# GregDMeyer/dynamite

Measured on AMD Instinct MI355X. Metric: matrix-free H|psi> Gamplitudes/s, random-field Heisenberg, higher is better.
Workload: dtype f64 (complex128)

## Files before the change

dynamite_amd/_lib.py:

```python
import ctypes as C
import os

import numpy as np

from . import build as _build

_HERE = os.path.dirname(os.path.abspath(__file__))

i64p = C.POINTER(C.c_int64)
f64p = C.POINTER(C.c_double)
vp = C.c_void_p


class Subspace(C.Structure):
    _fields_ = [("type", C.c_int32), ("L", C.c_int64), ("space", C.c_int64), ("k", C.c_int64),
                ("ld_nchoosek", C.c_int64), ("nchoosek", i64p), ("dim", C.c_int64),
                ("state_map", i64p), ("rmap_indices", i64p), ("rmap_states", i64p), ("vec_swizzle", C.c_int32),
                ("site_perm", C.POINTER(C.c_int8))]


class Partition(C.Structure):
    _fields_ = [("rank", C.c_int32), ("nranks", C.c_int32)]


# ... 17 lines not shown
LP_COUNT = 9
LP_NAMES = ["tile_real_k0", "tile_real", "tile_cplx", "tile_kvar_real", "tile_kvar_cplx", "gather_real",
            "gather_kvar_real", "gather_cplx", "gather_kvar_cplx"]
LP_KVAR, LP_CPLX, LP_GATHER = (3, 4, 6, 8), (2, 4, 7, 8), (5, 6, 7, 8)


class DevQuad(C.Structure):
    _fields_ = [("mask_tile", C.c_uint32), ("mask_loc", C.c_uint32), ("src", C.c_uint32),
                ("nslots", C.c_uint32), ("sign_tile", C.c_uint32 * 4), ("sign_ext", C.c_uint64 * 4),
                ("coeff", C.c_double * 4)]


class DevPass(C.Structure):
    _fields_ = [("nseg", C.c_int32), ("seg_off", C.c_int32 * MAXSEG), ("seg_len", C.c_int32 * MAXSEG),
                ("seg_pos", C.c_int32 * MAXSEG), ("nbseg", C.c_int32), ("bseg_off", C.c_int32 * MAXBSEG),
                ("bseg_len", C.c_int32 * MAXBSEG), ("bseg_pos", C.c_int32 * MAXBSEG),
                ("sign_base", C.c_uint64), ("accumulate", C.c_int32), ("need_tile", C.c_int32),
                ("has_diag", C.c_int32), ("cache_policy", C.c_int32), ("dext_begin", C.c_uint32), ("dext_end", C.c_uint32),
                ("dbucket", C.c_uint32 * (MAXR + 1)), ("loop", C.c_uint32 * (LP_COUNT + 1)),
                ("nquads", C.c_int32), ("n_eff", C.c_int32), ("quads", vp), ("dot_out", vp), ("zinit", vp), ("zscale", C.c_double), ("zinit2", vp), ("z2re", C.c_double), ("z2im", C.c_double),
                ("tile_bits", C.c_int32), ("log_rows", C.c_int32),
                ("swz_shift", C.c_int32), ("swz_xor_y", C.c_uint32), ("swz_xor_src", C.c_uint32), ("block_offset", C.c_uint32),
                ("pos_tmask", C.c_uint32), ("dtile", vp), ("tabs", vp), ("tabvals", vp), ("tab_loop", C.c_uint32 * 3),
                ("pad_tab", C.c_uint32), ("gbucket", C.c_uint32 * (MAXR + 1)), ("pad_g", C.c_uint32)]


class DevTab(C.Structure):
    _fields_ = [("mask_tile", C.c_uint32), ("mask_loc", C.c_uint32), ("src", C.c_uint32), ("first", C.c_uint32),
                ("z_tile", C.c_uint32), ("flags", C.c_uint32), ("tpos", C.c_uint32), ("twid", C.c_uint32),
                ("epos", C.c_uint32), ("ewid", C.c_uint32), ("z_ext", C.c_uint64), ("ik", C.c_uint64),
                ("ksign", C.c_uint32), ("nbits", C.c_uint32)]


class DevFlip(C.Structure):
    _fields_ = [("mask_tile", C.c_uint32), ("mask_pos", C.c_uint32), ("p0", C.c_uint32), ("p1", C.c_uint32),
                ("pad", C.c_uint32 * 2), ("c", C.c_double)]


FL_COUNT = 4
FL_NAMES = ["tile_thread", "tile_k", "gather_uniform", "gather_boundary"]


class Xfer(C.Structure):
    _fields_ = [("partner", C.c_int32), ("pass_id", C.c_int32), ("offset", C.c_int64), ("count", C.c_int64)]


MAT_DEFAULT, MAT_FORCE_GATHER, MAT_USE_GLDS, MAT_HOST_ONLY = 0, 1, 2, 4
# ... 46 lines not shown
    "dnm_mat_local_part_bits": (C.c_int, [vp, C.POINTER(C.c_int), C.POINTER(C.c_int)]),
    "dnm_mat_mult_window_local": (C.c_int, [vp, vp, vp, vp]),
    "dnm_mat_mult_window_remote": (C.c_int, [vp, vp, C.c_int64, C.c_int64, vp, vp]),
    "dnm_mat_window_local_rows": (C.c_int, [vp, C.c_int64, C.c_int64, C.c_int, C.c_int, C.POINTER(C.c_int64), C.POINTER(C.c_int), vp]),
    "dnm_mat_mult_window_rows": (C.c_int, [vp, vp, C.c_int64, C.c_int64, vp, C.c_int64, C.c_int64, vp]),
    "dnm_mat_destroy": (C.c_int, [vp]),
    "dnm_mat_sizes": (C.c_int, [vp, i64p, i64p, i64p, i64p]),
    "dnm_mat_precompute_diagonal": (C.c_int, [vp, vp]),
    "dnm_mat_get_diagonal": (C.c_int, [vp, f64p, vp]),
    "dnm_mat_mult": (C.c_int, [vp, vp, vp, vp]),
    "dnm_mat_norm_inf": (C.c_int, [vp, f64p, vp]),
    "dnm_mat_set_norm": (C.c_int, [vp, C.c_double]),
    "dnm_mat_plan_describe": (C.c_int, [vp, C.c_char_p, C.c_size_t]),
    "dnm_mat_plan_launches": (C.c_int, [vp, C.POINTER(C.c_int)]),
    "dnm_mat_plan_counts": (C.c_int, [vp] + [C.POINTER(C.c_int)] * 6),
    "dnm_mat_export_dtile": (C.c_int, [vp, C.c_int, C.c_int, f64p, C.c_int64]),
    "dnm_mat_export_tabs": (C.c_int, [vp, C.c_int, C.c_int, vp, C.c_size_t, C.c_int, C.POINTER(C.c_int), f64p, C.c_int64, i64p]),
    "dnm_mat_export_pass": (C.c_int, [vp, C.c_int, C.c_int, vp, C.c_size_t, vp, C.c_size_t, C.c_int,
                                      C.POINTER(C.c_int)]),
    "dnm_mat_export_flip": (C.c_int, [vp, C.c_int, C.c_int, vp, C.c_size_t, C.c_int, C.POINTER(C.c_int),
                                      C.POINTER(C.c_uint32), f64p]),
    "dnm_mat_export_flip_pass": (C.c_int, [vp, C.c_int, C.c_int, vp, C.c_size_t, vp, C.c_size_t, C.c_int,
                                           C.POINTER(C.c_int), f64p, C.c_int64, i64p]),
    "dnm_mat_ownership": (C.c_int, [vp, i64p, i64p]),
    "dnm_mat_column_window": (C.c_int, [vp, i64p, i64p, vp]),
    "dnm_mat_column_chunks": (C.c_int, [vp, C.c_int, C.POINTER(C.c_uint8), C.c_int64, vp]),
    "dnm_mat_mult_window": (C.c_int, [vp, vp, C.c_int64, C.c_int64, vp, vp]),
    "dnm_mat_exchange_plan": (C.c_int, [vp, C.POINTER(C.c_int), C.POINTER(Xfer), C.POINTER(C.c_int),
                                        C.POINTER(Xfer)]),
    "dnm_mat_mult_dot": (C.c_int, [vp, vp, vp, f64p, vp]),
    "dnm_mat_mult_lanczos": (C.c_int, [vp, vp, vp, vp, C.c_double, f64p, vp]),
    "dnm_mat_mult_local": (C.c_int, [vp, vp, vp, vp]),
    "dnm_mat_mult_remote": (C.c_int, [vp, C.c_int32, vp, vp, vp]),
    "dnm_vec_set": (C.c_int, [vp, C.c_int64, C.c_double, C.c_double, vp]),
    "dnm_vec_copy": (C.c_int, [vp, vp, C.c_int64, vp]),
    "dnm_vec_scale": (C.c_int, [vp, C.c_int64, C.c_double, C.c_double, vp]),
    "dnm_vec_axpby": (C.c_int, [vp, vp, C.c_int64, C.c_double, C.c_double, C.c_double, C.c_double, vp]),
    "dnm_vec_dot": (C.c_int, [vp, vp, C.c_int64, f64p, vp]),
    "dnm_vec_norm2": (C.c_int, [vp, C.c_int64, f64p, vp]),
    "dnm_vec_set_random": (C.c_int, [vp, C.c_int64, C.c_uint64, C.c_int64, vp]),
    "dnm_vec_mdot": (C.c_int, [vp, C.c_int64, C.c_int, vp, C.c_int64, f64p, vp]),
    "dnm_vec_maxpy": (C.c_int, [vp, vp, C.c_int64, C.c_int, C.c_int64, f64p, vp]),
    "dnm_vec_basis_update": (C.c_int, [vp, C.c_int64, C.c_int, C.c_int, C.c_int64, f64p, vp]),
    "dnm_workspace_bytes": (C.c_int, [C.POINTER(C.c_size_t)]),
    "dnm_release_workspace": (C.c_int, []),
    "dnm_mat_is_real_packed": (C.c_int, [C.c_void_p, C.POINTER(C.c_int)]),
# ... 77 lines not shown
```

dynamite_amd/csrc/mat.cpp:

```cpp
#include "passes.h"
#include "vec_api.h"
#include "row_fused.h"

#include <algorithm>
#include <cstring>

namespace dnm {

static thread_local std::string g_err;

void set_error(const char *fmt, ...) {
  char buf[1024];
  va_list ap;
  va_start(ap, fmt);
  vsnprintf(buf, sizeof(buf), fmt, ap);
  va_end(ap);
  g_err = buf;
}

int DevBuf::alloc(size_t nbytes) {
  release();
  if (nbytes == 0) nbytes = 16;
  DNM_HIP(hipMalloc(&p, nbytes));
  bytes = nbytes;
// ... 98 lines not shown
      dev.state_map = (const int64_t *)d_smap.p;
      dev.rmap_states = (const int64_t *)d_rstates.p;
      if (!rind.empty()) {
        DNM_TRY(d_rind.upload(rind.data(), rind.size() * 8));
        dev.rmap_indices = (const int64_t *)d_rind.p;
      }
      if (!bucket.empty()) {
        DNM_TRY(d_bucket.upload(bucket.data(), bucket.size() * 8));
        dev.bucket = (const int64_t *)d_bucket.p;
      }
    }
  }
  return 0;
}

template <class T>
static int upload_to(DevBuf &buf, const std::vector<T> &v, const T **dev) {
  DNM_TRY(buf.upload(v.data(), v.size() * sizeof(T)));
  *dev = (const T *)buf.p;
  return 0;
}
int PassRecords::upload() {
  DNM_TRY(upload_to(d_quads, quads, &desc.quads));
  if (!dtile.empty()) DNM_TRY(upload_to(d_dtile, dtile, &desc.dtile));
  if (!tabs.empty()) DNM_TRY(upload_to(d_tabs, tabs, &desc.tabs));
  if (!tabs.empty()) DNM_TRY(upload_to(d_tabvals, tabvals, &desc.tabvals));
  if (is_reduced) DNM_TRY(upload_to(d_flips, flips.empty() ? std::vector<DevFlip>(1) : flips, &flip.recs));
  return 0;
}

static hipStream_t S(void *stream) { return (hipStream_t)stream; }

struct PassCall {
  const void *zinit = nullptr, *zinit2 = nullptr;
  double zscale = 0.0, z2re = 0.0, z2im = 0.0;
  double *dot_out = nullptr;
  uint32_t block_offset = 0;
  unsigned nparts = 1;
};

static int launch_pass(const dnm_mat *A, const PassOnDevice &p, const PassCall &c, const void *x, void *y,
                       const void *xr, hipStream_t st) {
  DevPass d = p.runs().desc;
  d.zinit = c.zinit; d.zscale = c.zscale;
  d.zinit2 = c.zinit2; d.z2re = c.z2re; d.z2im = c.z2im;
  d.dot_out = c.dot_out;
  d.block_offset = c.block_offset;
// ... 6 lines not shown
}

static int export_lookup(const dnm_mat *A, int remote, int idx, const PassOnDevice **p) {
  DNM_CHECK(A, "null argument");
  const auto &v = remote ? A->remote_passes : A->local_passes;
  DNM_CHECK(idx >= 0 && idx < (int)v.size(), "pass index out of range");
  *p = v[idx].get();
  return 0;
}
template <class T>
static int export_copy(const std::vector<T> &v, void *out, size_t item, int64_t room, const char *type, const char *full,
                       bool strict = false) {
  if (!out || (v.empty() && !strict)) return 0;
  DNM_CHECK(item == sizeof(T), "%s size mismatch (%zu vs %zu)", type, item, sizeof(T));
  DNM_CHECK(room >= (int64_t)v.size(), "%s buffer too small", full);
  if (!v.empty()) memcpy(out, v.data(), v.size() * sizeof(T));
  return 0;
}
static int export_records(const PassRecords &r, void *desc_out, size_t desc_bytes, void *quads_out, size_t quad_bytes,
                          int max_quads, int *nquads, bool strict) {
  *nquads = (int)r.quads.size();
  if (desc_out) {
    DNM_CHECK(desc_bytes == sizeof(DevPass), "DevPass size mismatch (%zu vs %zu)", desc_bytes, sizeof(DevPass));
    memcpy(desc_out, &r.desc, sizeof(DevPass));
  }
  return export_copy(r.quads, quads_out, quad_bytes, max_quads, "DevQuad", "record", strict);
}

}

using namespace dnm;

namespace dnm {
std::vector<ScMask> sc_masks(const std::vector<int64_t> &masks, const std::vector<int64_t> &mask_offsets,
                             const std::vector<int64_t> &signs, const std::vector<double> &rcoef, int L, bool xparity) {
  std::vector<ScMask> scm(masks.size());
  for (size_t mi = 0; mi < masks.size(); ++mi) {
    ScMask &e = scm[mi];
    memset(&e, 0, sizeof(e));
    const uint64_t mask = (uint64_t)masks[mi];
    e.dead = __builtin_popcountll(mask) & 1;
    if (xparity && L >= 3 && __builtin_popcountll(mask) == L - 2 && !((mask >> (L - 1)) & 1ull)) {
      const uint64_t miss = ~mask & ((((uint64_t)1 << (L - 1)) - 1));
      const int i = __builtin_ctzll(miss);
      const uint64_t pairbits = ((uint64_t)1 << i) | ((uint64_t)1 << (L - 1));
      bool local = true;
      for (int64_t t = mask_offsets[mi]; t < mask_offsets[mi + 1]; ++t)
// ... 565 lines not shown
    if (cfg.diag_last < 0) cfg.diag_last = cfg.swz ? 1 : 0;
    if (cfg.window_first < 0) {
      int nl = A->op.n;
      for (int r = A->nranks; r > 1; r >>= 1) --nl;
      cfg.window_first = (cfg.swz && nl >= 25) ? 1 : 0;
    }
    if (!tile_config_supported(cfg.B, cfg.logR)) {
      set_error("unsupported tile configuration B=%d logR=%d", cfg.B, cfg.logR);
      return 1;
    }
    DNM_TRY(make_plan(A->op, A->rank, A->nranks, cfg, &A->plan));
    if (flags & DNM_MAT_FORCE_GATHER) A->plan.use_tiled = false;
    DNM_CHECK(!A->real_packed || A->plan.use_tiled, "real-packed operators run on the tiled kernel only (vector too small)");
    if (A->nranks > 1 && !A->plan.use_tiled) {
      A->plan.remote.clear();
      A->plan.sends.clear();
    }
    if (A->plan.use_tiled) {
      DNM_TRY(build_passes(*A, A->plan.local, &A->local_passes));
      DNM_TRY(build_passes(*A, A->plan.remote, &A->remote_passes));
      decide_flip_bonds(A.get());
      for (size_t i = 0; i < A->plan.local.size(); ++i)
        DNM_TRY(build_flip_pass(*A, A->plan.local[i], A->local_passes[i].get()));
      if (!A->host_only)
        for (auto *v : {&A->local_passes, &A->remote_passes})
          for (auto &p : *v) DNM_TRY(p->runs().upload());
    }
  }
  *out = A.release();
  return 0;
}

int dnm_mat_destroy(dnm_mat *A) {
  delete A;
  return 0;
}

int dnm_mat_set_exchange(dnm_mat *A, int scheme, int *chosen) {
  DNM_CHECK(A && chosen, "null argument");
  DNM_CHECK(scheme == DNM_EXCHANGE_AUTO || scheme == DNM_EXCHANGE_PARTNER || scheme == DNM_EXCHANGE_TRANSPOSE,
            "unknown exchange scheme %d", scheme);
  delete A->tr_lo; delete A->tr_hi;
  A->tr_lo = A->tr_hi = nullptr;
  A->tr_f = -1;
  *chosen = DNM_EXCHANGE_PARTNER;
  const int P = A->nranks;
// ... 603 lines not shown
  }
  const int nb = norm_num_blocks(A->rows_local);
  DNM_TRY(A->scratch.alloc((size_t)nb * sizeof(double)));
  DNM_TRY(launch_norm(A->dmsc, A->left.dev, A->right.dev, A->rows_local, A->row0,
                      (double *)A->scratch.p, S(stream)));
  std::vector<double> h(nb);
  DNM_TRY(dnm_memcpy_d2h(h.data(), A->scratch.p, (size_t)nb * sizeof(double), stream));
  double best = 0.0;
  for (double v : h) best = std::max(best, v);
  if (A->nranks == 1) A->nrm = best;
  *nrm = best;
  return 0;
}

int dnm_mat_set_norm(dnm_mat *A, double nrm) {
  DNM_CHECK(A, "null matrix");
  A->nrm = nrm;
  return 0;
}

int dnm_mat_plan_describe(const dnm_mat *A, char *buf, size_t buflen) {
  DNM_CHECK(A && buf && buflen, "null argument");
  std::string s;
  if (A->hypercube) s = A->plan.describe(A->op);
  else if (A->use_sc3) {
    const Sc3Tab &T = A->sc3->ly->host;
    char tmp[512];
    if (A->sc3->tiled && A->sc3->graph)
      snprintf(tmp, sizeof tmp, "SpinConserve two-pass kernels on a bond graph, internal layout [T %d | W %d | Lo %d]: "
               "window pass (%zu workgroups, %d hops in LDS, %d gathered) then lo pass (%zu workgroups, %d hops in LDS, "
               "%d gathered), diagonal %s, coefficients %s\n", T.t, T.w, T.a, A->sc3->permB.size(), A->sc3->op.nldsB,
               A->sc3->op.ngatB, A->sc3->permA.size() / 8, A->sc3->op.nldsA, A->sc3->op.ngatA,
               A->sc3->diag_mode == 2 ? "on the fly" : (A->sc3->diag_mode == 1 ? "cached" : "none"),
               A->sc3->sym ? "real symmetric" : "complex");
    else if (A->sc3->tiled)
      snprintf(tmp, sizeof tmp, "SpinConserve two-pass kernels, internal layout [T %d | W %d | Lo %d]: window pass (%zu "
               "workgroups, %d bonds in LDS, %d gathered) then lo pass (%zu workgroups, %d bonds in LDS, %d gathered), "
               "diagonal %s, coefficients %s\n", T.t, T.w, T.a, A->sc3->permB.size(), T.w - 1,
               __builtin_popcountll(A->sc3->op.bondsB), A->sc3->permA.size() / 8, T.a - 1,
               __builtin_popcountll(A->sc3->op.bondsA),
               A->sc3->diag_mode == 2 ? "on the fly" : (A->sc3->diag_mode == 1 ? "cached" : "none"),
               A->sc3->sym ? "real symmetric" : "complex");
    else
      snprintf(tmp, sizeof tmp, "SpinConserve row kernel, internal layout [T %d | W %d | Lo %d] (positions by table)\n",
               T.t, T.w, T.a);
    s = tmp;
  } else if (A->sc_pair)
// ... 45 lines not shown
                        int *nflips, uint32_t *loops_out, double *dconst) {
  const PassOnDevice *p;
  DNM_CHECK(nflips, "null argument");
  DNM_TRY(export_lookup(A, remote, idx, &p));
  *nflips = p->reduced ? (int)p->reduced->flips.size() : -1;
  if (!p->reduced) return 0;
  if (loops_out) memcpy(loops_out, p->reduced->flip.loop, sizeof(p->reduced->flip.loop));
  if (dconst) *dconst = p->reduced->flip.dconst;
  return export_copy(p->reduced->flips, flips_out, flip_bytes, max_flips, "DevFlip", "record");
}

int dnm_mat_export_flip_pass(const dnm_mat *A, int remote, int idx, void *desc_out, size_t desc_bytes, void *quads_out,
                             size_t quad_bytes, int max_quads, int *nquads, double *dtile_out, int64_t max_dtile,
                             int64_t *ndtile) {
  const PassOnDevice *p;
  DNM_CHECK(nquads && ndtile, "null argument");
  DNM_TRY(export_lookup(A, remote, idx, &p));
  DNM_CHECK(p->reduced, "the pass has no flip-flop form");
  *ndtile = (int64_t)p->reduced->dtile.size();
  DNM_TRY(export_records(*p->reduced, desc_out, desc_bytes, quads_out, quad_bytes, max_quads, nquads, false));
  return export_copy(p->reduced->dtile, dtile_out, sizeof(double), max_dtile, "double", "table");
}

int dnm_mat_plan_counts(const dnm_mat *A, int *n_local_passes, int *n_remote_passes, int *tiled,
                        int *B, int *logR, int *n_loc) {
  DNM_CHECK(A, "null matrix");
  if (n_local_passes) *n_local_passes = (int)A->local_passes.size();
  if (n_remote_passes) *n_remote_passes = (int)A->remote_passes.size();
  if (tiled) *tiled = (A->hypercube && A->plan.use_tiled) ? 1 : 0;
  if (B) *B = A->plan.cfg.B;
  if (logR) *logR = A->plan.cfg.logR;
  if (n_loc) *n_loc = A->plan.n_loc;
  return 0;
}

int dnm_mat_plan_launches(const dnm_mat *A, int *n) {
  DNM_CHECK(A && n, "null argument");
  *n = (A->hypercube && A->plan.use_tiled) ? (int)A->local_passes.size() : 1;
  return 0;
}

}

dnm_mat::~dnm_mat() {
  delete tr_lo;
  delete tr_hi;
// ... 2 lines not shown
```

dynamite_amd/csrc/mat.h:

```cpp
#pragma once

#include <memory>
#include <vector>

#include "kernels.h"
#include "plan.h"
#include "sc3.h"
#include "subspace.h"

namespace dnm {

struct DevBuf {
  void *p = nullptr;
  size_t bytes = 0;
  DevBuf() = default;
  DevBuf(const DevBuf &) = delete;
  DevBuf &operator=(const DevBuf &) = delete;
  ~DevBuf() { release(); }
  int alloc(size_t nbytes);
  int upload(const void *host, size_t nbytes);
  void release();
};

struct SubOwned {
  SubView host{};
  SubView dev{};
  std::vector<int64_t> nck, smap, rind, rstates, bucket;
  DevBuf d_nck, d_smap, d_rind, d_rstates, d_bucket;
  int init(const dnm_subspace *s, bool want_device);
};

struct PassRecords {
  DevPass desc{};
  std::vector<DevQuad> quads;
  std::vector<double> dtile;
  std::vector<DevTab> tabs;
  std::vector<double> tabvals;
  bool is_reduced = false;
  std::vector<DevFlip> flips;
  DevFlipPass flip{};
  DevBuf d_quads, d_dtile, d_tabs, d_tabvals, d_flips;
  int upload();
};

struct PassOnDevice {
  PassRecords whole;
  std::unique_ptr<PassRecords> reduced;
  PassRecords &runs() { return reduced ? *reduced : whole; }
  const PassRecords &runs() const { return reduced ? *reduced : whole; }
  int partner = -1;
  int n_eff = 0;
  int64_t y_off = 0, src_off = 0;
};

struct FlipBond {
  bool ok = false;
  bool exch = false;
  int b0 = 0, b1 = 0;
  double c = 0.0;
};

int rdm_release_scratch();

}
// ... 50 lines not shown
```

dynamite_amd/csrc/matvec_kernels.hip:

```cpp
#include <algorithm>
#include <cstdint>
#include <cstdlib>

#include "kernels.h"

namespace dnm {

typedef double2 c128;

#define GLOBAL_AS __attribute__((address_space(1)))
#define LDS_AS __attribute__((address_space(3)))

typedef double d2v __attribute__((ext_vector_type(2)));

typedef const __attribute__((address_space(4))) DevQuad CQuad;

__device__ __forceinline__ void store_through(c128 *p, double re, double im) {
  d2v v = {re, im};
  asm volatile("global_store_dwordx4 %0, %1, off sc1\n\ts_nop 1" ::"v"(p), "v"(v) : "memory");
}
__device__ __forceinline__ void store_streaming(c128 *p, double re, double im) {
  d2v v = {re, im};
  __builtin_nontemporal_store(v, reinterpret_cast<d2v *>(p));
}
// ... 336 lines not shown
  }
}

#ifndef DNM_WAVES_4ROWS
#define DNM_WAVES_4ROWS 8
#endif
constexpr int tile_waves_per_simd(int B, int LOGR, bool TAB = false) {
  if (TAB) {
    int nt = 1 << (B - LOGR);
    int blocks = (160 * 1024) / (16 << B);
    if (blocks < 1) blocks = 1;
    int w = blocks * nt / 256;
    const int cap = LOGR <= 2 ? 8 : 4;
    return w < 1 ? 1 : (w > cap ? cap : w);
  }
  int nt = 1 << (B - LOGR);
  int blocks = (160 * 1024) / (16 << B);
  if (blocks < 1) blocks = 1;
  int w = blocks * nt / 256;
  const int cap = LOGR <= 2 ? DNM_WAVES_4ROWS : 4;
  return w < 1 ? 1 : (w > cap ? cap : w);
}

template <int B, int LOGR, bool GLDS, int GV, bool PACK, bool TAB, bool FLIP>
__device__ __forceinline__ void tile_pass_body(const DevPass &P, const c128 *__restrict__ x, c128 *__restrict__ y,
                                               const c128 *__restrict__ xr, const DevFlipPass &FP) {
  constexpr int R = 1 << LOGR;
  constexpr int LOGNT = B - LOGR;
  constexpr uint32_t NT = 1u << LOGNT;
  extern __shared__ __attribute__((aligned(16))) unsigned char smem[];
  c128 *tile = reinterpret_cast<c128 *>(smem);

  const uint32_t tid = threadIdx.x;
  DNM_PH(0, 0);
  const uint32_t base = deposit<MAXBSEG>(blockIdx.x + P.block_offset, P.nbseg, P.bseg_off, P.bseg_len, P.bseg_pos);
  const uint32_t dep_t = deposit<MAXSEG>(tid, P.nseg, P.seg_off, P.seg_len, P.seg_pos);
  const uint64_t sbase = P.sign_base | (uint64_t)base;

  const uint32_t skw = (uint32_t)P.swz_shift;
  auto lay = [skw](uint32_t v) -> uint32_t { return skw ? (v ^ (((v >> skw) & ((1u << (skw - 4)) - 1u)) << 4)) : v; };
  RowAddr<R> RA;
  RA.t4 = lay(dep_t) << 4;
  RA.upos = lay(base);
  RA.tmask = P.pos_tmask;
#pragma unroll
  for (int k = 0; k < R; ++k) RA.kpos[k] = lay(deposit<MAXSEG>((uint32_t)k << LOGNT, P.nseg, P.seg_off, P.seg_len, P.seg_pos));
  const uint32_t yx = P.swz_xor_y;
// ... 67 lines not shown

#define DNM_LOOP(LP, KV, CX, GA, KZ) \
  apply_records<R, LOGNT, KV, CX, GA, KZ, PACK>(quads, P.loop[LP], P.loop[LP + 1], ar, ai, tile, RA, x, xr, tid, sbase, skw, P.swz_xor_src)
  if constexpr (GV >= 1) {
    DNM_LOOP(LP_GATHER_REAL, false, false, true, false);
    DNM_LOOP(LP_GATHER_KVAR_REAL, true, false, true, false);
    DNM_LOOP(LP_GATHER_CPLX, false, true, true, false);
    DNM_LOOP(LP_GATHER_KVAR_CPLX, true, true, true, false);
  }
#undef DNM_LOOP
  if constexpr (FLIP)
    flip_gathers<R, LOGNT>((CFlip *)FP.recs, FP.loop[FL_GATHER_U], FP.loop[FL_GATHER_B], FP.loop[FL_GATHER_B + 1], ar, ai, RA,
                           x, tid, sbase);
  c128 *tabl = nullptr;
  if constexpr (TAB) {
    __shared__ __attribute__((aligned(16))) unsigned char tabl_mem[TABL_ENTRIES * 16];
    tabl = reinterpret_cast<c128 *>(tabl_mem);
  }
  if constexpr (TAB)
    apply_tabs<R, LOGNT, true>((CTab *)P.tabs, (const c128 *)P.tabvals, P.tab_loop[1], P.tab_loop[2], ar, ai, tile, RA, x, xr,
                               tid, sbase, skw, P.swz_xor_src, tabl);
  DNM_PH(2, 1);

  double dext = 0.0;
  if (P.has_diag) {
    const uint32_t lane = tid & 63u;
    const uint32_t nterm = (P.dext_end - P.dext_begin) * 4u;
    for (uint32_t t0 = 0; t0 < nterm; t0 += 64u) {
      const uint32_t t = t0 + lane;
      double v = 0.0;
      if (t < nterm) {
        CQuad &Q = quads[P.dext_begin + (t >> 2)];
        const uint32_t j = t & 3u;
        const uint32_t p = (uint32_t)__popcll(sbase & Q.sign_ext[j]) & 1u;
        v = flip_sign(Q.coeff[j], p);
      }
      dext += v;
    }
#pragma unroll
    for (int off = 32; off > 0; off >>= 1) dext += __shfl_xor(dext, off, 64);
  }
  double *cg = nullptr;
  if constexpr (TAB) {
    __shared__ double cg_mem[MAXDGROUPS];
    cg = cg_mem;
    if (P.has_diag) {
      const uint32_t lane = tid & 63u, g0 = P.gbucket[0], g1 = P.gbucket[R];
      for (uint32_t g = g0 + (tid >> 6); g < g1; g += (NT >> 6)) {
        const uint32_t q0 = quads[g].mask_loc, nterm = quads[g].src * 4u;
        double v = 0.0;
        for (uint32_t t0 = 0; t0 < nterm; t0 += 64u) {
          const uint32_t t = t0 + lane;
          if (t < nterm) {
            CQuad &Q = quads[q0 + (t >> 2)];
            const uint32_t j = t & 3u;
            v += flip_sign(Q.coeff[j], (uint32_t)__popcll(sbase & Q.sign_ext[j]) & 1u);
          }
        }
#pragma unroll
        for (int off = 32; off > 0; off >>= 1) v += __shfl_xor(v, off, 64);
        if (lane == 0) cg[g - g0] = v;
      }
    }
  }
  auto diag_part2 = [&]() {
  if (P.has_diag) {
    double D[R];
#pragma unroll
    for (int j = 0; j < R; ++j) D[j] = 0.0;
    D[0] = dext;
    if constexpr (FLIP) D[0] += FP.dconst;
    double dtab[R];
    if (P.dtile) {
#pragma unroll
      for (int k = 0; k < R; ++k) dtab[k] = P.dtile[tid + k * NT];
    }
#pragma unroll
    for (int j = 0; j < R; ++j)
      for (uint32_t q = P.dbucket[j]; q < P.dbucket[j + 1]; ++q) {
        const uint32_t ns = quads[q].nslots;
        double v = slot_amp(quads[q], 0, tid, sbase);
        if (ns > 1) v += slot_amp(quads[q], 1, tid, sbase);
        if (ns > 2) v += slot_amp(quads[q], 2, tid, sbase);
        if (ns > 3) v += slot_amp(quads[q], 3, tid, sbase);
        D[j] += v;
      }
    if constexpr (TAB) {
      const uint32_t g0 = P.gbucket[0];
#pragma unroll
// ... 96 lines not shown
      dn += __shfl_xor(dn, off, 64);
    }
    __shared__ double dred[3 * (NT / 64 > 0 ? NT / 64 : 1)];
    if ((tid & 63u) == 0) {
      dred[3 * (tid >> 6)] = dr;
      dred[3 * (tid >> 6) + 1] = di;
      dred[3 * (tid >> 6) + 2] = dn;
    }
    __syncthreads();
    if (tid == 0) {
      double sr = 0.0, si = 0.0, sn = 0.0;
      for (uint32_t w = 0; w < NT / 64; ++w) {
        sr += dred[3 * w];
        si += dred[3 * w + 1];
        sn += dred[3 * w + 2];
      }
      P.dot_out[3 * (size_t)blockIdx.x] = sr;
      P.dot_out[3 * (size_t)blockIdx.x + 1] = si;
      P.dot_out[3 * (size_t)blockIdx.x + 2] = sn;
    }
  }
}

template <int B, int LOGR, bool GLDS, int GV, bool PACK = false, bool TAB = false>
__global__ void __launch_bounds__(1 << (B - LOGR), tile_waves_per_simd(B, LOGR, TAB))
tile_pass_kernel(const DevPass P, const c128 *__restrict__ x, c128 *__restrict__ y,
                 const c128 *__restrict__ xr) {
  tile_pass_body<B, LOGR, GLDS, GV, PACK, TAB, false>(P, x, y, xr, DevFlipPass{});
}

template <int B, int LOGR, bool GLDS>
__global__ void __launch_bounds__(1 << (B - LOGR), tile_waves_per_simd(B, LOGR, false))
tile_pass_flip_kernel(const DevPass P, const DevFlipPass FP, const c128 *__restrict__ x, c128 *__restrict__ y,
                      const c128 *__restrict__ xr) {
  tile_pass_body<B, LOGR, GLDS, 1, false, false, true>(P, x, y, xr, FP);
}

#ifdef DNM_PHASE_TIMING
}
extern "C" int dnm_debug_phase_buffer(void *buf) {
  unsigned long long *p = (unsigned long long *)buf;
  return hipMemcpyToSymbol(HIP_SYMBOL(dnm::g_phase_buf), &p, sizeof(p)) == hipSuccess ? 0 : 1;
}
namespace dnm {
#endif

template <int B, int LOGR>
static int launch_cfg(const DevPass &P, bool glds, int n_loc, const void *x, void *y,
                      const void *xr, hipStream_t st, unsigned nparts, const DevFlipPass *F) {
  constexpr int NT = 1 << (B - LOGR);
  static const size_t lds_req = []() {
    const char *e = knob("DNM_LDS_KB");
    return e ? (size_t)atoi(e) * 1024 : (size_t)0;
  }();
  const size_t lds = std::max(((size_t)16 << B), lds_req);
  const unsigned grid = (1u << (n_loc - B)) / nparts;
  const int gv = (P.cache_policy & 32) ? 1 : 0;
  using kern_t = void (*)(const DevPass, const c128 *, c128 *, const c128 *);
  kern_t k = nullptr;
  const bool pack = (P.cache_policy & 256) != 0;
  const bool tab = P.tab_loop[2] > 0 || P.gbucket[MAXR] > P.gbucket[0];
  if (F) {
    DNM_CHECK(!pack && !tab && gv == 1, "internal: flip-flop records in a pass that cannot run them");
    using fkern_t = void (*)(const DevPass, const DevFlipPass, const c128 *, c128 *, const c128 *);
    fkern_t fk = glds ? tile_pass_flip_kernel<B, LOGR, true> : tile_pass_flip_kernel<B, LOGR, false>;
    static size_t fattr_done[2] = {0, 0};
    if (fattr_done[glds ? 1 : 0] < lds) {
      DNM_HIP(hipFuncSetAttribute((const void *)fk, hipFuncAttributeMaxDynamicSharedMemorySize, (int)lds));
      fattr_done[glds ? 1 : 0] = lds;
    }
    hipLaunchKernelGGL(fk, dim3(grid), dim3(NT), lds, st, P, *F, (const c128 *)x, (c128 *)y, (const c128 *)xr);
    DNM_HIP(hipGetLastError());
    return 0;
  }
  if (pack) k = tile_pass_kernel<B, LOGR, false, 1, true>;
  else if (tab) k = tile_pass_kernel<B, LOGR, false, 1, false, true>;
  else if (glds) k = tile_pass_kernel<B, LOGR, true, 1>;
  else if (gv == 0) k = tile_pass_kernel<B, LOGR, false, 0>;
  else k = tile_pass_kernel<B, LOGR, false, 1>;
  static size_t attr_done[6] = {0, 0, 0, 0, 0, 0};
  const int slot = pack ? 4 : (tab ? 5 : (glds ? 3 : gv));
  if (attr_done[slot] < lds) {
    DNM_HIP(hipFuncSetAttribute((const void *)k, hipFuncAttributeMaxDynamicSharedMemorySize, (int)lds));
    attr_done[slot] = lds;
  }
  hipLaunchKernelGGL(k, dim3(grid), dim3(NT), lds, st, P, (const c128 *)x, (c128 *)y, (const c128 *)xr);
  DNM_HIP(hipGetLastError());
  return 0;
}

bool tile_config_supported(int B, int logR) {
  switch (B * 16 + logR) {
    case 10 * 16 + 2: case 11 * 16 + 2: case 12 * 16 + 2:
    case 8 * 16 + 2: case 10 * 16 + 3: case 10 * 16 + 4: case 11 * 16 + 3: case 11 * 16 + 4:
    case 12 * 16 + 3: case 12 * 16 + 4: case 13 * 16 + 3: case 13 * 16 + 4:
      return true;
  }
  return false;
}

int launch_tile_pass(const DevPass &P, int B, int logR, bool glds, int n_loc, const void *x,
                     void *y, const void *xr, hipStream_t st, unsigned nparts, const DevFlipPass *F) {
  DNM_CHECK(n_loc >= B, "tile larger than the local vector");
  switch (B * 16 + logR) {
// ... 857 lines not shown
```

dynamite_amd/csrc/passes.cpp:

```cpp
#include "passes.h"

#include <algorithm>
#include <cstring>

namespace dnm {

int build_opform(const dnm_mat &A, OpForm *op) {
  const SubView &l = A.left.host, &r = A.right.host;
  const bool par = l.type == DNM_PARITY;
  const int n = par ? l.L - 1 : l.L;
  op->n = n;
  op->masks.clear();
  const uint64_t ones = n >= 64 ? ~0ull : (((uint64_t)1 << n) - 1);
  for (size_t mi = 0; mi < A.masks.size(); ++mi) {
    const uint64_t mask = (uint64_t)A.masks[mi];
    if (par && (parity64(mask) != (l.space ^ r.space))) continue;
    RowMask rm;
    rm.mask = par ? (mask >> 1) : mask;
    for (int64_t t = A.mask_offsets[mi]; t < A.mask_offsets[mi + 1]; ++t) {
      const uint64_t sg = (uint64_t)A.signs[t];
      RowTerm rt;
      rt.is_imag = parity64(mask & sg);
      double c = A.real_coeffs[t];
      uint64_t s2 = sg;
// ... 537 lines not shown
      DNM_CHECK(it != dterms.end(), "internal: an exchange without a ZZ term on its pair");
      if (it->coeff == a) dterms.erase(it);
      else it->coeff -= a;
      dconst -= a;
      diag_changed = true;
    }
  if (!diag_changed && std::find(skip.begin(), skip.end(), 1) == skip.end()) return 0;
  std::unique_ptr<PassRecords> r(new PassRecords());
  r->is_reduced = true;
  r->desc = d;
  DNM_TRY(emit_records(A, ps, *r, dm ? &dterms : nullptr, skip));
  DNM_CHECK(r->tabs.empty() && r->desc.gbucket[MAXR] == r->desc.gbucket[0],
            "internal: the flip-flop form of a pass has table records or grouped diagonal terms");
  for (int c = 0; c < FL_COUNT; ++c) {
    r->flip.loop[c] = (uint32_t)r->flips.size();
    r->flips.insert(r->flips.end(), fl[c].begin(), fl[c].end());
  }
  r->flip.loop[FL_COUNT] = (uint32_t)r->flips.size();
  r->flip.dconst = dconst;
  out->reduced = std::move(r);
  return 0;
}

}
```

dynamite_amd/csrc/passes.h:

```cpp
#pragma once

#include "mat.h"

namespace dnm {

int build_opform(const dnm_mat &A, OpForm *op);
int pack_opform(OpForm *op);
int build_pass(const dnm_mat &A, const PassSpec &ps, PassOnDevice *out);
void decide_flip_bonds(dnm_mat *A);
int build_flip_pass(const dnm_mat &A, const PassSpec &ps, PassOnDevice *out);

}
```

dynamite_amd/csrc/plan.cpp:

```cpp
#include "plan.h"

#include <algorithm>
#include <cstdlib>
#include <sstream>

namespace dnm {

static int env_int(const char *name, int dflt) {
  const char *v = knob(name);
  if (!v) return dflt;
  return atoi(v);
}

PlanConfig plan_config_from_env() {
  PlanConfig c;
  c.B = env_int("DNM_TILE_BITS", c.B);
  c.logR = env_int("DNM_LOG_ROWS", c.logR);
  c.amin = env_int("DNM_AMIN", c.amin);
  c.mode = env_int("DNM_PLAN_MODE", c.mode);
  c.gbits = env_int("DNM_GBITS", c.gbits);
  c.gbits_window = env_int("DNM_GBITS_WINDOW", c.gbits_window);
  c.window_first = env_int("DNM_WINDOW_FIRST", c.window_first);
  c.Bw = env_int("DNM_TILE_BITS_WINDOW", c.Bw);
  c.logRw = env_int("DNM_LOG_ROWS_WINDOW", c.logRw);
// ... 278 lines not shown
    std::vector<Need> theirs;
    remote_needs(op, q, nl, B, &theirs);
    for (const Need &nd : theirs)
      if (nd.partner == rank) pl.sends.push_back({q, nd.src_off, (int64_t)1 << nd.n_eff});
  }
  return 0;
}

int make_plan(const OpForm &op, int rank, int nranks, const PlanConfig &cfg_in, Plan *out) {
  if (cfg_in.amin >= 0) return make_plan_with(op, rank, nranks, cfg_in, out);
  PlanConfig c4 = cfg_in;
  c4.amin = 4;
  DNM_TRY(make_plan_with(op, rank, nranks, c4, out));
  if (out->use_tiled && out->n_loc >= 29 && out->cfg.mode == 2 && !cfg_in.swz) {
    PlanConfig c6 = cfg_in;
    c6.amin = 6;
    Plan p6;
    DNM_TRY(make_plan_with(op, rank, nranks, c6, &p6));
    if (p6.local.size() <= out->local.size()) *out = p6;
  }
  return 0;
}

std::string Plan::describe(const OpForm &op) const {
  std::ostringstream os;
  os << "n=" << n << " n_loc=" << n_loc << " rank=" << rank << "/" << nranks
     << " tiled=" << (use_tiled ? 1 : 0) << " B=" << cfg.B << " logR=" << cfg.logR
     << " mode=" << cfg.mode << " masks=" << op.masks.size() << "\n";
  auto dump = [&](const char *kind, const PassSpec &ps, size_t i) {
    os << kind << " pass " << i << ":";
    if (ps.B != cfg.B || (ps.logR && ps.logR != cfg.logR)) os << " B=" << ps.B << " logR=" << (ps.logR ? ps.logR : cfg.logR);
    os << " segs";
    for (int j = 0; j < ps.nseg; ++j)
      os << " [" << ps.seg_pos[j] << "," << ps.seg_pos[j] + ps.seg_len[j] << ")";
    if (ps.glen) os << " xcd-group [" << ps.gpos << "," << ps.gpos + ps.glen << ")";
    os << " diag=" << ps.has_diag << " acc=" << ps.accumulate << " tile_masks=" << ps.tile_masks.size()
       << " gather_masks=" << ps.gather_masks.size();
    if (ps.partner >= 0)
      os << " partner=" << ps.partner << " rows [" << ps.y_off << ",+2^" << ps.n_eff << ") from partner offset "
         << ps.src_off;
    os << "\n";
  };
  for (size_t i = 0; i < local.size(); ++i) dump("local", local[i], i);
  for (size_t i = 0; i < remote.size(); ++i) dump("remote", remote[i], i);
  return os.str();
}

}
```

dynamite_amd/csrc/plan.h:

```cpp
#pragma once

#include <cstdint>
#include <string>
#include <vector>

#include "dnm_common.h"

namespace dnm {

constexpr int MAXSEG = 4;
constexpr int MAXBSEG = 8;
constexpr int MAXSRC = 8;
constexpr int MAXR = 16;

struct RowTerm {
  uint64_t sign;
  double coeff;
  int is_imag;
};

struct RowMask {
  uint64_t mask;
  std::vector<RowTerm> terms;
  bool zero_mask_offdiag = false;
// ... 59 lines not shown
  uint32_t dbucket[MAXR + 1];
  uint32_t loop[LP_COUNT + 1];
  int32_t nquads;
  int32_t n_eff;
  const DevQuad *quads;
  double *dot_out;
  const void *zinit;
  double zscale;
  const void *zinit2;
  double z2re, z2im;
  int32_t tile_bits;
  int32_t log_rows;
  int32_t swz_shift;
  uint32_t swz_xor_y, swz_xor_src;
  uint32_t block_offset;
  uint32_t pos_tmask;
  const double *dtile;
  const DevTab *tabs;
  const double *tabvals;
  uint32_t tab_loop[3];
  uint32_t pad_tab;
  uint32_t gbucket[MAXR + 1];
  uint32_t pad_g;
};
constexpr uint32_t MAXDGROUPS = 64;

struct DevFlip {
  uint32_t mask_tile;
  uint32_t mask_pos;
  uint32_t p0, p1;
  uint32_t pad[2];
  double c;
};
enum {
  FL_TILE_T = 0,
  FL_TILE_K,
  FL_GATHER_U,
  FL_GATHER_B,
  FL_COUNT
};
struct DevFlipPass {
  const DevFlip *recs;
  uint32_t loop[FL_COUNT + 1];
  uint32_t pad;
  double dconst;
};

struct PassSpec {
// ... 22 lines not shown
  int B = 12;
  int logR = -1;
  int amin = -1;
  int mode = 2;
  int gbits = -1;
  int Bw = 0, logRw = 0;
  int window_first = -1;
  int gbits_window = -1;
  int cache_policy = 226;
  int max_gather_span = 0;
  int diag_last = -1;
  int swz = 0;
};

struct Plan {
  int n = 0, n_loc = 0;
  int rank = 0, nranks = 1;
  PlanConfig cfg;
  std::vector<PassSpec> local;
  std::vector<PassSpec> remote;
  struct Send { int partner; int64_t offset, count; };
  std::vector<Send> sends;
  bool use_tiled = false;
  std::string describe(const OpForm &op) const;
};

PlanConfig plan_config_from_env();
int make_plan(const OpForm &op, int rank, int nranks, const PlanConfig &cfg, Plan *out);

}
```

include/dynamite_amd.h:

```cpp
#ifndef DYNAMITE_AMD_H
#define DYNAMITE_AMD_H

#include <stddef.h>
#include <stdint.h>

#ifdef __cplusplus
extern "C" {
#endif

const char *dnm_last_error(void);
int dnm_version(void);
int dnm_device_count(int *count);
int dnm_set_device(int device);
int dnm_malloc(void **dptr, size_t bytes);
int dnm_free(void *dptr);
int dnm_memcpy_h2d(void *dst, const void *src, size_t bytes, void *stream);
int dnm_memcpy_d2h(void *dst, const void *src, size_t bytes, void *stream);
int dnm_stream_synchronize(void *stream);

enum { DNM_FULL = 0, DNM_PARITY = 1, DNM_EXPLICIT = 2, DNM_SPIN_CONSERVE = 3 };

typedef struct dnm_subspace {
  int32_t type;
  int64_t L;
// ... 51 lines not shown
int dnm_mat_destroy(dnm_mat *A);
int dnm_mat_sizes(const dnm_mat *A, int64_t *M, int64_t *N, int64_t *m_local, int64_t *n_local);
int dnm_mat_precompute_diagonal(dnm_mat *A, void *stream);
int dnm_mat_get_diagonal(dnm_mat *A, double *diag_host, void *stream);
int dnm_mat_mult(dnm_mat *A, const void *x, void *y, void *stream);
int dnm_mat_norm_inf(dnm_mat *A, double *nrm, void *stream);
int dnm_mat_layouts(const dnm_mat *A, int *left, int *right);
int dnm_mat_is_real_packed(const dnm_mat *A, int *packed);
int dnm_mat_set_norm(dnm_mat *A, double nrm);
int dnm_mat_plan_describe(const dnm_mat *A, char *buf, size_t buflen);
int dnm_mat_plan_launches(const dnm_mat *A, int *n);
int dnm_mat_plan_counts(const dnm_mat *A, int *n_local_passes, int *n_remote_passes, int *tiled,
                        int *B, int *logR, int *n_loc);
int dnm_mat_export_dtile(const dnm_mat *A, int remote, int idx, double *out, int64_t n);
int dnm_mat_export_pass(const dnm_mat *A, int remote, int idx, void *desc_out, size_t desc_bytes,
                        void *quads_out, size_t quad_bytes, int max_quads, int *nquads);
int dnm_mat_export_tabs(const dnm_mat *A, int remote, int idx, void *tabs_out, size_t tab_bytes, int max_tabs, int *ntabs,
                        double *vals_out, int64_t max_vals, int64_t *nvals);
int dnm_mat_export_flip(const dnm_mat *A, int remote, int idx, void *flips_out, size_t flip_bytes, int max_flips,
                        int *nflips, uint32_t *loops_out, double *dconst);
int dnm_mat_export_flip_pass(const dnm_mat *A, int remote, int idx, void *desc_out, size_t desc_bytes, void *quads_out,
                             size_t quad_bytes, int max_quads, int *nquads, double *dtile_out, int64_t max_dtile,
                             int64_t *ndtile);

typedef struct {
  int32_t partner;
  int32_t pass_id;
  int64_t offset;
  int64_t count;
} dnm_xfer;
int dnm_mat_exchange_plan(const dnm_mat *A, int *nsend, dnm_xfer *sends ,
                          int *nrecv, dnm_xfer *recvs );
int dnm_mat_mult_dot(dnm_mat *A, const void *x, void *y, double *dot , void *stream);
int dnm_mat_mult_lanczos(dnm_mat *A, const void *x, void *y, const void *z, double b,
                         double *dot , void *stream);
int dnm_mat_mult_sub(dnm_mat *A, const void *x, void *y, const void *z, double b, void *stream);
int dnm_mat_fuses_init(const dnm_mat *A);
int dnm_mat_mult_sub2(dnm_mat *A, const void *x, void *y, const void *z, double b, const void *z2,
                      double c_re, double c_im, void *stream);
int dnm_mat_mult_local(dnm_mat *A, const void *x_local, void *y, void *stream);
int dnm_mat_mult_remote(dnm_mat *A, int32_t recv_index, const void *x_recv,
                        void *y, void *stream);

int dnm_mat_ownership(const dnm_mat *A, int64_t *row0, int64_t *m_local);
int dnm_mat_window_split(const dnm_mat *A, int *supported);
int dnm_mat_mult_local_part(dnm_mat *A, const void *x, void *y, int part, int nparts, void *stream);
// ... 121 lines not shown
```

Before: 68.12.

## Precompute per-block diagonal tables to replace on-the-fly diagonal evaluation

Adds a host-side precomputation of the diagonal's per-block external part (one value per tile block) and per-tile sections indexed by the parity of a few cross-term masks. The tile kernel then reads one block constant and one section entry per row instead of looping over diagonal terms with popcount and sign logic. This is meant to cut ALU and loop overhead in the diagonal phase. In exchange it uses extra device memory (up to 2^22 block entries plus up to 8 tile sections), adds build time, and adds more kernel template instances.

```diff
diff --git a/dynamite_amd/_lib.py b/dynamite_amd/_lib.py
--- a/dynamite_amd/_lib.py
+++ b/dynamite_amd/_lib.py
@@ -63,7 +63,8 @@
                 ("tile_bits", C.c_int32), ("log_rows", C.c_int32),
                 ("swz_shift", C.c_int32), ("swz_xor_y", C.c_uint32), ("swz_xor_src", C.c_uint32), ("block_offset", C.c_uint32),
                 ("pos_tmask", C.c_uint32), ("dtile", vp), ("tabs", vp), ("tabvals", vp), ("tab_loop", C.c_uint32 * 3),
-                ("pad_tab", C.c_uint32), ("gbucket", C.c_uint32 * (MAXR + 1)), ("pad_g", C.c_uint32)]
+                ("pad_tab", C.c_uint32), ("gbucket", C.c_uint32 * (MAXR + 1)), ("pad_g", C.c_uint32),
+                ("dblock", vp), ("dsel_n", C.c_uint32), ("pad_d", C.c_uint32), ("dsel_mask", C.c_uint64 * 3)]
 
 
 class DevTab(C.Structure):
@@ -156,6 +157,8 @@
                                       C.POINTER(C.c_uint32), f64p]),
     "dnm_mat_export_flip_pass": (C.c_int, [vp, C.c_int, C.c_int, vp, C.c_size_t, vp, C.c_size_t, C.c_int,
                                            C.POINTER(C.c_int), f64p, C.c_int64, i64p]),
+    "dnm_mat_export_diag_tables": (C.c_int, [vp, C.c_int, C.c_int, f64p, C.c_int64, i64p, f64p, C.c_int64, i64p,
+                                             C.POINTER(C.c_uint64), C.POINTER(C.c_int)]),
     "dnm_mat_ownership": (C.c_int, [vp, i64p, i64p]),
     "dnm_mat_column_window": (C.c_int, [vp, i64p, i64p, vp]),
     "dnm_mat_column_chunks": (C.c_int, [vp, C.c_int, C.POINTER(C.c_uint8), C.c_int64, vp]),
diff --git a/dynamite_amd/csrc/mat.cpp b/dynamite_amd/csrc/mat.cpp
--- a/dynamite_amd/csrc/mat.cpp
+++ b/dynamite_amd/csrc/mat.cpp
@@ -144,7 +144,8 @@
 }
 int PassRecords::upload() {
   DNM_TRY(upload_to(d_quads, quads, &desc.quads));
-  if (!dtile.empty()) DNM_TRY(upload_to(d_dtile, dtile, &desc.dtile));
+  if (!dtile.empty()) DNM_TRY(upload_to(d_dtile, dblock.empty() ? dtile : dtile_sections(), &desc.dtile));
+  if (!dblock.empty()) DNM_TRY(upload_to(d_dblock, dblock, &desc.dblock));
   if (!tabs.empty()) DNM_TRY(upload_to(d_tabs, tabs, &desc.tabs));
   if (!tabs.empty()) DNM_TRY(upload_to(d_tabvals, tabvals, &desc.tabvals));
   if (is_reduced) DNM_TRY(upload_to(d_flips, flips.empty() ? std::vector<DevFlip>(1) : flips, &flip.recs));
@@ -197,7 +198,11 @@
   *nquads = (int)r.quads.size();
   if (desc_out) {
     DNM_CHECK(desc_bytes == sizeof(DevPass), "DevPass size mismatch (%zu vs %zu)", desc_bytes, sizeof(DevPass));
-    memcpy(desc_out, &r.desc, sizeof(DevPass));
+    DevPass d = r.desc;
+    d.dblock = nullptr;
+    d.dsel_n = 0;
+    memset(d.dsel_mask, 0, sizeof(d.dsel_mask));
+    memcpy(desc_out, &d, sizeof(DevPass));
   }
   return export_copy(r.quads, quads_out, quad_bytes, max_quads, "DevQuad", "record", strict);
 }
@@ -809,6 +814,8 @@
       decide_flip_bonds(A.get());
       for (size_t i = 0; i < A->plan.local.size(); ++i)
         DNM_TRY(build_flip_pass(*A, A->plan.local[i], A->local_passes[i].get()));
+      for (auto *v : {&A->local_passes, &A->remote_passes})
+        for (auto &p : *v) DNM_TRY(build_diag_tables(*A, p.get()));
       if (!A->host_only)
         for (auto *v : {&A->local_passes, &A->remote_passes})
           for (auto &p : *v) DNM_TRY(p->runs().upload());
@@ -1458,7 +1465,13 @@
 int dnm_mat_plan_describe(const dnm_mat *A, char *buf, size_t buflen) {
   DNM_CHECK(A && buf && buflen, "null argument");
   std::string s;
-  if (A->hypercube) s = A->plan.describe(A->op);
+  if (A->hypercube) {
+    std::vector<std::string> notes[2];
+    const std::vector<std::unique_ptr<PassOnDevice>> *lists[2] = {&A->local_passes, &A->remote_passes};
+    for (int k = 0; k < 2; ++k)
+      for (const auto &p : *lists[k]) notes[k].push_back(p->runs().dblock.empty() ? "" : " diag_tables=1");
+    s = A->plan.describe(A->op, &notes[0], &notes[1]);
+  }
   else if (A->use_sc3) {
     const Sc3Tab &T = A->sc3->ly->host;
     char tmp[512];
@@ -1550,6 +1563,23 @@
   return export_copy(p->reduced->dtile, dtile_out, sizeof(double), max_dtile, "double", "table");
 }
 
+int dnm_mat_export_diag_tables(const dnm_mat *A, int remote, int idx, double *dblock_out, int64_t max_dblock,
+                               int64_t *ndblock, double *dtile_out, int64_t max_dtile, int64_t *ndtile,
+                               uint64_t *masks_out, int *nmasks) {
+  const PassOnDevice *p;
+  DNM_CHECK(ndblock && ndtile && nmasks, "null argument");
+  DNM_TRY(export_lookup(A, remote, idx, &p));
+  const PassRecords &r = p->runs();
+  const bool have = !r.dblock.empty();
+  *ndblock = (int64_t)r.dblock.size();
+  *ndtile = have ? (int64_t)r.dtile_sections().size() : 0;
+  *nmasks = have ? (int)r.desc.dsel_n : 0;
+  if (!have) return 0;
+  if (masks_out) memcpy(masks_out, r.desc.dsel_mask, sizeof(r.desc.dsel_mask));
+  DNM_TRY(export_copy(r.dblock, dblock_out, sizeof(double), max_dblock, "double", "table"));
+  return export_copy(r.dtile_sections(), dtile_out, sizeof(double), max_dtile, "double", "table");
+}
+
 int dnm_mat_plan_counts(const dnm_mat *A, int *n_local_passes, int *n_remote_passes, int *tiled,
                         int *B, int *logR, int *n_loc) {
   DNM_CHECK(A, "null matrix");
diff --git a/dynamite_amd/csrc/mat.h b/dynamite_amd/csrc/mat.h
--- a/dynamite_amd/csrc/mat.h
+++ b/dynamite_amd/csrc/mat.h
@@ -39,7 +39,9 @@
   bool is_reduced = false;
   std::vector<DevFlip> flips;
   DevFlipPass flip{};
-  DevBuf d_quads, d_dtile, d_tabs, d_tabvals, d_flips;
+  std::vector<double> dblock, dsect;
+  const std::vector<double> &dtile_sections() const { return dsect.empty() ? dtile : dsect; }
+  DevBuf d_quads, d_dtile, d_tabs, d_tabvals, d_flips, d_dblock;
   int upload();
 };
 
diff --git a/dynamite_amd/csrc/matvec_kernels.hip b/dynamite_amd/csrc/matvec_kernels.hip
--- a/dynamite_amd/csrc/matvec_kernels.hip
+++ b/dynamite_amd/csrc/matvec_kernels.hip
@@ -382,7 +382,7 @@
   return w < 1 ? 1 : (w > cap ? cap : w);
 }
 
-template <int B, int LOGR, bool GLDS, int GV, bool PACK, bool TAB, bool FLIP>
+template <int B, int LOGR, bool GLDS, int GV, bool PACK, bool TAB, bool FLIP, bool DT>
 __device__ __forceinline__ void tile_pass_body(const DevPass &P, const c128 *__restrict__ x, c128 *__restrict__ y,
                                                const c128 *__restrict__ xr, const DevFlipPass &FP) {
   constexpr int R = 1 << LOGR;
@@ -496,8 +496,14 @@
                                tid, sbase, skw, P.swz_xor_src, tabl);
   DNM_PH(2, 1);
 
+  static_assert(!DT || (!TAB && !PACK), "no table-driven diagonal on the TAB and PACK instances");
   double dext = 0.0;
-  if (P.has_diag) {
+  uint32_t dsec = 0;
+  if constexpr (DT) {
+    dext = ((const __attribute__((address_space(4))) double *)P.dblock)[blockIdx.x + P.block_offset];
+#pragma unroll
+    for (int i = 0; i < MAXDSEL; ++i) dsec |= ((uint32_t)__popcll(sbase & P.dsel_mask[i]) & 1u) << i;
+  } else if (P.has_diag) {
     const uint32_t lane = tid & 63u;
     const uint32_t nterm = (P.dext_end - P.dext_begin) * 4u;
     for (uint32_t t0 = 0; t0 < nterm; t0 += 64u) {
@@ -538,7 +544,16 @@
     }
   }
   auto diag_part2 = [&]() {
-  if (P.has_diag) {
+  if constexpr (DT) {
+    const double *__restrict__ dsect = P.dtile + ((size_t)dsec << B) + tid;
+#pragma unroll
+    for (int k = 0; k < R; ++k) {
+      const double Dk = dext + dsect[k * NT];
+      c128 xs = tile[tid + k * NT];
+      ar[k] = fma(Dk, xs.x, ar[k]);
+      ai[k] = fma(Dk, xs.y, ai[k]);
+    }
+  } else if (P.has_diag) {
     double D[R];
 #pragma unroll
     for (int j = 0; j < R; ++j) D[j] = 0.0;
@@ -681,18 +696,18 @@
   }
 }
 
-template <int B, int LOGR, bool GLDS, int GV, bool PACK = false, bool TAB = false>
+template <int B, int LOGR, bool GLDS, int GV, bool PACK = false, bool TAB = false, bool DT = false>
 __global__ void __launch_bounds__(1 << (B - LOGR), tile_waves_per_simd(B, LOGR, TAB))
 tile_pass_kernel(const DevPass P, const c128 *__restrict__ x, c128 *__restrict__ y,
                  const c128 *__restrict__ xr) {
-  tile_pass_body<B, LOGR, GLDS, GV, PACK, TAB, false>(P, x, y, xr, DevFlipPass{});
-}
-
-template <int B, int LOGR, bool GLDS>
+  tile_pass_body<B, LOGR, GLDS, GV, PACK, TAB, false, DT>(P, x, y, xr, DevFlipPass{});
+}
+
+template <int B, int LOGR, bool GLDS, bool DT = false>
 __global__ void __launch_bounds__(1 << (B - LOGR), tile_waves_per_simd(B, LOGR, false))
 tile_pass_flip_kernel(const DevPass P, const DevFlipPass FP, const c128 *__restrict__ x, c128 *__restrict__ y,
                       const c128 *__restrict__ xr) {
-  tile_pass_body<B, LOGR, GLDS, 1, false, false, true>(P, x, y, xr, FP);
+  tile_pass_body<B, LOGR, GLDS, 1, false, false, true, DT>(P, x, y, xr, FP);
 }
 
 #ifdef DNM_PHASE_TIMING
@@ -719,14 +734,18 @@
   kern_t k = nullptr;
   const bool pack = (P.cache_policy & 256) != 0;
   const bool tab = P.tab_loop[2] > 0 || P.gbucket[MAXR] > P.gbucket[0];
+  const bool dt = P.has_diag && P.dblock != nullptr;
+  DNM_CHECK(!dt || (!pack && !tab && gv == 1), "internal: a table-driven diagonal in a pass that cannot run it");
   if (F) {
     DNM_CHECK(!pack && !tab && gv == 1, "internal: flip-flop records in a pass that cannot run them");
     using fkern_t = void (*)(const DevPass, const DevFlipPass, const c128 *, c128 *, const c128 *);
-    fkern_t fk = glds ? tile_pass_flip_kernel<B, LOGR, true> : tile_pass_flip_kernel<B, LOGR, false>;
-    static size_t fattr_done[2] = {0, 0};
-    if (fattr_done[glds ? 1 : 0] < lds) {
+    fkern_t fk = dt ? (glds ? tile_pass_flip_kernel<B, LOGR, true, true> : tile_pass_flip_kernel<B, LOGR, false, true>)
+                    : (glds ? tile_pass_flip_kernel<B, LOGR, true> : tile_pass_flip_kernel<B, LOGR, false>);
+    static size_t fattr_done[4] = {0, 0, 0, 0};
+    const int fslot = (glds ? 1 : 0) + (dt ? 2 : 0);
+    if (fattr_done[fslot] < lds) {
       DNM_HIP(hipFuncSetAttribute((const void *)fk, hipFuncAttributeMaxDynamicSharedMemorySize, (int)lds));
-      fattr_done[glds ? 1 : 0] = lds;
+      fattr_done[fslot] = lds;
     }
     hipLaunchKernelGGL(fk, dim3(grid), dim3(NT), lds, st, P, *F, (const c128 *)x, (c128 *)y, (const c128 *)xr);
     DNM_HIP(hipGetLastError());
@@ -734,11 +753,12 @@
   }
   if (pack) k = tile_pass_kernel<B, LOGR, false, 1, true>;
   else if (tab) k = tile_pass_kernel<B, LOGR, false, 1, false, true>;
+  else if (dt) k = glds ? tile_pass_kernel<B, LOGR, true, 1, false, false, true> : tile_pass_kernel<B, LOGR, false, 1, false, false, true>;
   else if (glds) k = tile_pass_kernel<B, LOGR, true, 1>;
   else if (gv == 0) k = tile_pass_kernel<B, LOGR, false, 0>;
   else k = tile_pass_kernel<B, LOGR, false, 1>;
-  static size_t attr_done[6] = {0, 0, 0, 0, 0, 0};
-  const int slot = pack ? 4 : (tab ? 5 : (glds ? 3 : gv));
+  static size_t attr_done[8] = {0, 0, 0, 0, 0, 0, 0, 0};
+  const int slot = pack ? 4 : (tab ? 5 : (dt ? (glds ? 7 : 6) : (glds ? 3 : gv)));
   if (attr_done[slot] < lds) {
     DNM_HIP(hipFuncSetAttribute((const void *)k, hipFuncAttributeMaxDynamicSharedMemorySize, (int)lds));
     attr_done[slot] = lds;
diff --git a/dynamite_amd/csrc/passes.cpp b/dynamite_amd/csrc/passes.cpp
--- a/dynamite_amd/csrc/passes.cpp
+++ b/dynamite_amd/csrc/passes.cpp
@@ -583,4 +583,53 @@
   return 0;
 }
 
-}
+int build_diag_tables(const dnm_mat &A, PassOnDevice *out) {
+  PassRecords &r = out->runs();
+  DevPass &d = r.desc;
+  const char *e = knob("DNM_DIAG_BLOCK_TABLE");
+  if (!d.has_diag || (e && e[0] == '0') || r.dtile.empty() || A.op.packed || !(d.cache_policy & 32)) return 0;
+  if (!r.tabs.empty() || d.gbucket[MAXR] > d.gbucket[0]) return 0;
+  const int B = d.tile_bits, R = 1 << d.log_rows, nbb = d.n_eff - B;
+  if (nbb < 0 || nbb > MAXDBLOCK_BITS) return 0;
+  std::vector<uint64_t> sel;
+  for (uint32_t q = d.dbucket[0]; q < d.dbucket[R]; ++q)
+    for (uint32_t j = 0; j < r.quads[q].nslots; ++j) {
+      const uint64_t m = r.quads[q].sign_ext[j];
+      if (m && std::find(sel.begin(), sel.end(), m) == sel.end()) sel.push_back(m);
+    }
+  if ((int)sel.size() > MAXDSEL) return 0;
+  r.dblock.resize((size_t)1 << nbb);
+  for (uint32_t b = 0; b < ((uint32_t)1 << nbb); ++b) {
+    uint64_t base = 0;
+    for (int j = 0; j < d.nbseg; ++j)
+      base |= (uint64_t)((b >> d.bseg_off[j]) & ((1u << d.bseg_len[j]) - 1u)) << d.bseg_pos[j];
+    const uint64_t sbase = d.sign_base | base;
+    double v = r.is_reduced ? r.flip.dconst : 0.0;
+    for (uint32_t q = d.dext_begin; q < d.dext_end; ++q)
+      for (uint32_t j = 0; j < r.quads[q].nslots; ++j)
+        v += parity64(sbase & r.quads[q].sign_ext[j]) ? -r.quads[q].coeff[j] : r.quads[q].coeff[j];
+    r.dblock[b] = v;
+  }
+  d.dsel_n = (uint32_t)sel.size();
+  for (size_t i = 0; i < sel.size(); ++i) d.dsel_mask[i] = sel[i];
+  if (!sel.empty()) {
+    const size_t T = (size_t)1 << B;
+    r.dsect.resize(T << sel.size());
+    for (size_t s = 0; s < ((size_t)1 << sel.size()); ++s) {
+      double *sec = r.dsect.data() + s * T;
+      std::copy(r.dtile.begin(), r.dtile.end(), sec);
+      for (uint32_t q = d.dbucket[0]; q < d.dbucket[R]; ++q)
+        for (uint32_t j = 0; j < r.quads[q].nslots; ++j) {
+          const DevQuad &Q = r.quads[q];
+          uint32_t po = 0;
+          for (size_t i = 0; i < sel.size(); ++i)
+            if (sel[i] == Q.sign_ext[j]) po = (uint32_t)(s >> i) & 1u;
+          for (uint32_t tc = 0; tc < (uint32_t)T; ++tc)
+            sec[tc] += ((__builtin_popcount(tc & Q.sign_tile[j]) ^ po) & 1) ? -Q.coeff[j] : Q.coeff[j];
+        }
+    }
+  }
+  return 0;
+}
+
+}
diff --git a/dynamite_amd/csrc/passes.h b/dynamite_amd/csrc/passes.h
--- a/dynamite_amd/csrc/passes.h
+++ b/dynamite_amd/csrc/passes.h
@@ -9,5 +9,6 @@
 int build_pass(const dnm_mat &A, const PassSpec &ps, PassOnDevice *out);
 void decide_flip_bonds(dnm_mat *A);
 int build_flip_pass(const dnm_mat &A, const PassSpec &ps, PassOnDevice *out);
+int build_diag_tables(const dnm_mat &A, PassOnDevice *out);
 
 }
diff --git a/dynamite_amd/csrc/plan.cpp b/dynamite_amd/csrc/plan.cpp
--- a/dynamite_amd/csrc/plan.cpp
+++ b/dynamite_amd/csrc/plan.cpp
@@ -324,12 +324,13 @@
   return 0;
 }
 
-std::string Plan::describe(const OpForm &op) const {
+std::string Plan::describe(const OpForm &op, const std::vector<std::string> *local_notes,
+                           const std::vector<std::string> *remote_notes) const {
   std::ostringstream os;
   os << "n=" << n << " n_loc=" << n_loc << " rank=" << rank << "/" << nranks
      << " tiled=" << (use_tiled ? 1 : 0) << " B=" << cfg.B << " logR=" << cfg.logR
      << " mode=" << cfg.mode << " masks=" << op.masks.size() << "\n";
-  auto dump = [&](const char *kind, const PassSpec &ps, size_t i) {
+  auto dump = [&](const char *kind, const PassSpec &ps, size_t i, const std::vector<std::string> *notes) {
     os << kind << " pass " << i << ":";
     if (ps.B != cfg.B || (ps.logR && ps.logR != cfg.logR)) os << " B=" << ps.B << " logR=" << (ps.logR ? ps.logR : cfg.logR);
     os << " segs";
@@ -341,10 +342,11 @@
     if (ps.partner >= 0)
       os << " partner=" << ps.partner << " rows [" << ps.y_off << ",+2^" << ps.n_eff << ") from partner offset "
          << ps.src_off;
+    if (notes && i < notes->size()) os << (*notes)[i];
     os << "\n";
   };
-  for (size_t i = 0; i < local.size(); ++i) dump("local", local[i], i);
-  for (size_t i = 0; i < remote.size(); ++i) dump("remote", remote[i], i);
+  for (size_t i = 0; i < local.size(); ++i) dump("local", local[i], i, local_notes);
+  for (size_t i = 0; i < remote.size(); ++i) dump("remote", remote[i], i, remote_notes);
   return os.str();
 }
 
diff --git a/dynamite_amd/csrc/plan.h b/dynamite_amd/csrc/plan.h
--- a/dynamite_amd/csrc/plan.h
+++ b/dynamite_amd/csrc/plan.h
@@ -105,8 +105,14 @@
   uint32_t pad_tab;
   uint32_t gbucket[MAXR + 1];
   uint32_t pad_g;
+  const double *dblock;
+  uint32_t dsel_n;
+  uint32_t pad_d;
+  uint64_t dsel_mask[3];
 };
 constexpr uint32_t MAXDGROUPS = 64;
+constexpr int MAXDSEL = 3;
+constexpr int MAXDBLOCK_BITS = 22;
 
 struct DevFlip {
   uint32_t mask_tile;
@@ -175,7 +181,8 @@
   struct Send { int partner; int64_t offset, count; };
   std::vector<Send> sends;
   bool use_tiled = false;
-  std::string describe(const OpForm &op) const;
+  std::string describe(const OpForm &op, const std::vector<std::string> *local_notes = nullptr,
+                       const std::vector<std::string> *remote_notes = nullptr) const;
 };
 
 PlanConfig plan_config_from_env();
diff --git a/include/dynamite_amd.h b/include/dynamite_amd.h
--- a/include/dynamite_amd.h
+++ b/include/dynamite_amd.h
@@ -97,6 +97,9 @@
 int dnm_mat_export_flip_pass(const dnm_mat *A, int remote, int idx, void *desc_out, size_t desc_bytes, void *quads_out,
                              size_t quad_bytes, int max_quads, int *nquads, double *dtile_out, int64_t max_dtile,
                              int64_t *ndtile);
+int dnm_mat_export_diag_tables(const dnm_mat *A, int remote, int idx, double *dblock_out, int64_t max_dblock,
+                               int64_t *ndblock, double *dtile_out, int64_t max_dtile, int64_t *ndtile,
+                               uint64_t *masks_out, int *nmasks);
 
 typedef struct {
   int32_t partner;
```

Result: faster. 69.64 (median of 6 runs) (+2.2%).
